# SenseTime-FVG/OpenDWM

Hardware: AMD Instinct MI355X
Metric: denoise-steps/sec (6-view x16f 448x256), SD-3.5 CTSD (higher is better)
Workload: dtype bf16; 1 GPU; CTSD SD-3.5 MMDiT (24 joint blocks, 13 dual, 6 cross-view + 12 temporal VT blocks, point-wise temporal + ImageAdapter), 6 views x 16 frames x 448x256 px (latents [1,16,6,16,32,56]), CFG g=4 -> model batch 2, 154 text tokens, FlowMatch-Euler; one replica per GPU; layers=24, finite=True, residual_stream=fp32 (GEMM operands and activations bf16), variant=text+layout (ImageAdapter recomputed every step, pointwise temporal)

## Files before the change

### include/dwm_hip.h

```cpp
#ifndef DWM_HIP_H
#define DWM_HIP_H

#include <stdint.h>

#ifdef __cplusplus
extern "C" {
#endif

#define DWM_OK 0
#define DWM_EINVAL (-1)
#define DWM_EALIGN (-2)
#define DWM_EUNSUPPORTED (-3)

#define DWM_ABI_VERSION 18
int dwm_abi_version(void);
const char* dwm_source_hash(void);

enum {
    DWM_EPI_PLAIN = 0,
    DWM_EPI_GEGLU = 1,
    DWM_EPI_RESID = 2,
    DWM_EPI_RMSHEAD = 3
};
enum { DWM_ACT_NONE = 0, DWM_ACT_GELU_TANH = 1, DWM_ACT_SILU = 2, DWM_ACT_RELU = 3 };

typedef struct dwm_rowmap2d {
    int64_t rw, rh;
    int64_t rpitch, ipitch;
    int64_t origin;
    int64_t xstep;
} dwm_rowmap2d;

typedef struct dwm_gemm_args {
    const void* A;  int64_t lda;
    const void* W;
    const void* bias;
    void* C;        int64_t ldc;
    int64_t M, N, K;
    int32_t epilogue;
    int32_t act;
    const void* gate; int64_t ld_gate; int64_t rows_per_gate;
    const void* res;  int64_t ld_res;  int64_t res_mod;
    const void* blend; int64_t ld_blend;
    const float* alpha; int64_t rows_per_alpha;
    const void* rms_w; int64_t rms_ncols; float rms_eps;
    int32_t reserved;
    dwm_rowmap2d a_map;
    dwm_rowmap2d c_map;
    int32_t ntaps; int32_t k_per_tap;
    int64_t tap_shift[27];
    void* workspace; int64_t workspace_bytes; int32_t split_k;
    void* C32; int64_t ldc32;
    int32_t tile;
} dwm_gemm_args;

int dwm_gemm_bf16(const dwm_gemm_args* args, void* stream);
int64_t dwm_gemm4w_launches(void);
int64_t dwm_gemm4w_launches_general(void);

typedef struct dwm_gemm_tn_args {
    const void* A; int64_t lda;
    const void* B; int64_t ldb; int64_t b_rows;
    void* out; int64_t ldo;
    int64_t M, N, C;
    int32_t ntaps; int32_t split_k;
    int64_t tap_shift[27];
    void* workspace; int64_t workspace_bytes;
} dwm_gemm_tn_args;
int dwm_gemm_tn(const dwm_gemm_tn_args* args, void* stream);

typedef struct dwm_attn_args {
    const void *q0, *k0, *v0; int64_t ld0;
    const void *q1, *k1, *v1; int64_t ld1;
    void* o0; int64_t ldo0;
    void* o1; int64_t ldo1;
    int64_t L0, L1;
    int64_t n_problems;
    int32_t heads; int32_t head_dim;
    float scale;
    int32_t mask_mode;
    int64_t pdiv[3], pmod[3], pstride[3];
    int64_t ldiv[2], lstride[3];
    const uint8_t* mask; int64_t mask_G; int64_t group_size; int64_t p_per_mask;
    int32_t variant;
    int32_t cross;
    float* lse;
} dwm_attn_args;

int dwm_attention_fwd(const dwm_attn_args* args, void* stream);
int64_t dwm_attn_stream_launches(void);

typedef struct dwm_attn_bwd_args {
    dwm_attn_args fwd;
    const void *do0, *do1;
    void *dq0, *dk0, *dv0; int64_t ld_d0;
    void *dq1, *dk1, *dv1; int64_t ld_d1;
    float* delta;
} dwm_attn_bwd_args;
int dwm_attention_bwd(const dwm_attn_bwd_args* args, void* stream);

int dwm_debug_tr_probe(const int32_t* offs, int16_t* out, void* stream);

typedef struct dwm_layernorm_args {
    const void* x; int64_t ldx;
    void* y;       int64_t ldy;
    void* y2;      int64_t ldy2;
    void* xsum;    int64_t ldxsum;
    int64_t rows; int32_t D; float eps;
    const void* weight; const void* bias;
    const void* scale;  const void* shift;  int64_t ld_mod;  int64_t rows_per_mod;
    const void* scale2; const void* shift2;
// ... 189 lines not shown
```

### opendwm_amd/_lib.py

```python
from __future__ import annotations

import ctypes as C
import os

HERE = os.path.dirname(os.path.abspath(__file__))
LIB_PATH = os.environ.get("DWM_HIP_LIB") or os.path.join(HERE, "libdwm_hip.so")
ABI_VERSION = 18

EPI_PLAIN, EPI_GEGLU, EPI_RESID, EPI_RMSHEAD = 0, 1, 2, 3
ACT_NONE, ACT_GELU_TANH, ACT_SILU, ACT_RELU = 0, 1, 2, 3

_i64, _i32, _f32, _vp = C.c_int64, C.c_int32, C.c_float, C.c_void_p


class RowMap2D(C.Structure):
    _fields_ = [("rw", _i64), ("rh", _i64), ("rpitch", _i64), ("ipitch", _i64), ("origin", _i64), ("xstep", _i64)]


class GemmTnArgs(C.Structure):
    _fields_ = [
        ("A", _vp), ("lda", _i64), ("B", _vp), ("ldb", _i64), ("b_rows", _i64), ("out", _vp), ("ldo", _i64),
        ("M", _i64), ("N", _i64), ("C", _i64), ("ntaps", _i32), ("split_k", _i32), ("tap_shift", _i64 * 27),
        ("workspace", _vp), ("workspace_bytes", _i64),
    ]
# ... 44 lines not shown
        ("weight", _vp), ("bias", _vp),
        ("scale", _vp), ("shift", _vp), ("ld_mod", _i64), ("rows_per_mod", _i64),
        ("scale2", _vp), ("shift2", _vp),
        ("addvec", _vp), ("ld_add", _i64), ("rows_per_add", _i64),
    ]


class GnImgMap(C.Structure):
    _fields_ = [("iv", _i64), ("pn", _i64), ("s_ihi", _i64), ("s_ilo", _i64), ("s_phi", _i64)]


class GnZMap(C.Structure):
    _fields_ = [("mod", _vp), ("ld_mod", _i64), ("frames", _i32), ("videos", _i32), ("h", _i32), ("w", _i32),
                ("shift", _i32), ("zt", _i32 * 32)]


class FrameMix(C.Structure):
    _fields_ = [("n_out", _i32), ("f0", _i32 * 64), ("f1", _i32 * 64), ("w0", _f32 * 64), ("w1", _f32 * 64)]


class BlockPermuteArgs(C.Structure):
    _fields_ = [("src", C.c_void_p), ("dst", C.c_void_p), ("block_bytes", C.c_int64), ("n", C.c_int64 * 4), ("sstride", C.c_int64 * 4)]


class RowCombineArgs(C.Structure):
    _fields_ = [
        ("a", _vp), ("lda", _i64), ("gate_a", _vp), ("ld_gate_a", _i64), ("rows_per_gate_a", _i64),
        ("coef_a", _vp), ("rows_per_coef_a", _i64), ("b", _vp), ("ldb", _i64),
        ("coef_b", _vp), ("rows_per_coef_b", _i64), ("out", _vp), ("ldo", _i64), ("rows", _i64), ("ncols", _i64),
    ]


class LayerNormBwdArgs(C.Structure):
    _fields_ = [
        ("x", _vp), ("ldx", _i64), ("addvec", _vp), ("ld_add", _i64), ("rows_per_add", _i64),
        ("dy", _vp), ("lddy", _i64), ("dy2", _vp), ("lddy2", _i64),
        ("dx", _vp), ("lddx", _i64), ("accumulate", _i32),
        ("rows", _i64), ("D", _i32), ("eps", _f32), ("weight", _vp),
        ("scale", _vp), ("scale2", _vp), ("ld_mod", _i64), ("rows_per_mod", _i64),
        ("dgamma", _vp), ("dbeta", _vp), ("dgamma2", _vp), ("dbeta2", _vp), ("ld_grad", _i64), ("grad_per_group", _i32),
    ]


class AdamW8Item(C.Structure):
    _fields_ = [("p", _vp), ("g", _vp), ("m_q", _vp), ("m_absmax", _vp), ("v_q", _vp), ("v_absmax", _vp), ("p_bf16", _vp), ("n", _i64)]


SIGNATURES = {
    "dwm_abi_version": (_i32, []),
    "dwm_source_hash": (C.c_char_p, []),
    "dwm_gemm_bf16": (_i32, [C.POINTER(GemmArgs), _vp]),
    "dwm_gemm4w_launches": (_i64, []),
    "dwm_gemm4w_launches_general": (_i64, []),
    "dwm_attn_stream_launches": (_i64, []),
    "dwm_gemm_tn": (_i32, [C.POINTER(GemmTnArgs), _vp]),
    "dwm_attention_fwd": (_i32, [C.POINTER(AttnArgs), _vp]),
    "dwm_attention_bwd": (_i32, [C.POINTER(AttnBwdArgs), _vp]),
    "dwm_debug_tr_probe": (_i32, [_vp, _vp, _vp]),
    "dwm_layernorm": (_i32, [C.POINTER(LayerNormArgs), _vp]),
    "dwm_layernorm_x32": (_i32, [C.POINTER(LayerNormArgs), _vp]),
    "dwm_rmsnorm_heads": (_i32, [_vp, _i64, _i64, _i64, _vp, _f32, _vp]),
    "dwm_silu": (_i32, [_vp, _vp, _i64, _vp]),
    "dwm_timestep_sinusoid": (_i32, [_vp, _i64, _i32, _vp, _vp]),
    "dwm_patchify": (_i32, [_vp, _i32, _i64, _i32, _i32, _i32, _i32, _vp, _i64, _vp]),
    "dwm_unpatchify": (_i32, [_vp, _i64, _i64, _i32, _i32, _i32, _i32, _vp, _vp]),
    "dwm_cfg_euler_step": (_i32, [_vp, _vp, _vp, _i64, _f32, _f32, _vp]),
    "dwm_cfg_euler_step_grouped": (_i32, [_vp, _vp, _vp, _i64, _f32, _vp, _i64, _vp]),
    "dwm_cast_f32_to_bf16": (_i32, [_vp, _vp, _i64, _vp]),
    "dwm_gemm_f32": (_i32, [C.POINTER(GemmArgs), _vp]),
    "dwm_layernorm_f32": (_i32, [C.POINTER(LayerNormArgs), _vp]),
    "dwm_groupnorm_silu_f32": (_i32, [_vp, _vp, _i64, _i64, _i32, _i32, _f32, _vp, _vp, _i32, _vp, C.POINTER(RowMap2D), C.POINTER(GnImgMap), _vp]),
    "dwm_upsample2_padded_f32": (_i32, [_vp, _vp, _i64, _i32, _i32, _i32, _vp]),
    "dwm_pad_tokens_f32": (_i32, [_vp, _vp, _i64, _i32, C.POINTER(RowMap2D), _vp]),
    "dwm_softmax_rows_f32": (_i32, [_vp, _vp, _i64, _i32, _i64, _f32, _vp]),
    "dwm_unshuffle_tokens_f32": (_i32, [_vp, _i64, _i32, _i32, _i32, _i32, _vp, _i64, _vp]),
    "dwm_avgpool2_tokens_f32": (_i32, [_vp, _i64, _i32, _i32, _i32, _vp, _vp]),
    "dwm_cfg_multistep_f32": (_i32, [_vp, _vp, _vp, _vp, _i64, _f32, _f32, _f32, _f32, _f32, _f32, _vp]),
    "dwm_attention_f32": (_i32, [C.POINTER(AttnArgs), _vp]),
    "dwm_silu_f32": (_i32, [_vp, _vp, _i64, _vp]),
    "dwm_timestep_sinusoid_f32": (_i32, [_vp, _i64, _i32, _vp, _vp]),
    "dwm_patchify_f32": (_i32, [_vp, _i64, _i32, _i32, _i32, _i32, _vp, _i64, _vp]),
    "dwm_unpatchify_f32": (_i32, [_vp, _i64, _i64, _i32, _i32, _i32, _i32, _vp, _vp]),
    "dwm_cfg_euler_step_f32": (_i32, [_vp, _vp, _vp, _i64, _f32, _f32, _vp, _i64, _vp]),
    "dwm_ray_features": (_i32, [_vp, _i64, _i32, _i32, _vp, _i64, _vp]),
    "dwm_ray_features_f32": (_i32, [_vp, _i64, _i32, _i32, _vp, _i64, _vp]),
    "dwm_frame_affine": (_i32, [_vp, _vp, _vp, _vp, _vp, _i64, _i64, _vp]),
    "dwm_cfg_ddim_step": (_i32, [_vp, _i32, _i32, _vp, _vp, _vp, _vp, _vp, _i64, _i64, _f32, _i32, _f32, _i32, _vp]),
    "dwm_cfg_multistep": (_i32, [_vp, _vp, _vp, _vp, _i64, _f32, _f32, _f32, _f32, _f32, _f32, _vp]),
    "dwm_unshuffle_tokens": (_i32, [_vp, _i32, _i64, _i32, _i32, _i32, _i32, _vp, _i64, _vp]),
    "dwm_avgpool2_tokens": (_i32, [_vp, _i64, _i32, _i32, _i32, _vp, _vp]),
    "dwm_add_inplace": (_i32, [_vp, _vp, _i64, _vp]),
    "dwm_add_f32_inplace": (_i32, [_vp, _vp, _i64, _vp]),
    "dwm_add_f32_f32_inplace": (_i32, [_vp, _vp, _i64, _vp]),
    "dwm_groupnorm_silu": (_i32, [_vp, _vp, _i64, _i64, _i32, _i32, _f32, _vp, _vp, _i32, _vp, C.POINTER(RowMap2D), _vp]),
    "dwm_groupnorm_silu_mapped": (_i32, [_vp, _vp, _i64, _i64, _i32, _i32, _f32, _vp, _vp, _i32, _vp, C.POINTER(RowMap2D), C.POINTER(GnImgMap), _vp]),
    "dwm_upsample2_padded": (_i32, [_vp, _vp, _i64, _i32, _i32, _i32, _vp]),
    "dwm_pad_tokens": (_i32, [_vp, _vp, _i64, _i32, C.POINTER(RowMap2D), _vp]),
    "dwm_groupnorm_stats_floats": (_i64, [_i64, _i64, _i32]),
    "dwm_groupnorm_spatial": (_i32, [_vp, _vp, _i64, _i64, _i32, _i32, _f32, _vp, _vp, _i32, _vp, C.POINTER(RowMap2D),
                                     C.POINTER(GnImgMap), C.POINTER(GnZMap), _vp]),
    "dwm_frame_mix_bf16": (_i32, [_vp, _vp, _i64, C.POINTER(FrameMix), _vp]),
    "dwm_frame_mix_f32": (_i32, [_vp, _vp, _i64, C.POINTER(FrameMix), _vp]),
    "dwm_groupnorm_spatial_f32": (_i32, [_vp, _vp, _i64, _i64, _i32, _i32, _f32, _vp, _vp, _i32, _vp, C.POINTER(RowMap2D),
                                         C.POINTER(GnImgMap), C.POINTER(GnZMap), _vp]),
    "dwm_softmax_rows": (_i32, [_vp, _vp, _i64, _i32, _i64, _f32, _vp]),
    "dwm_transpose_bf16": (_i32, [_vp, _i64, _i64, _i64, _vp, _i64, _i64, _vp]),
# ... 70 lines not shown
```

### opendwm_amd/build.py

```python
from __future__ import annotations

import os
import shutil
import subprocess
import sys
from concurrent.futures import ThreadPoolExecutor

HERE = os.path.dirname(os.path.abspath(__file__))
CSRC = os.path.join(HERE, "csrc")
INCLUDE = os.path.join(os.path.dirname(HERE), "include")
LIB = os.path.join(HERE, "libdwm_hip.so")
SOURCES = ["gemm_bf16.hip", "gemm_bf16_4w.hip", "gemm_tn.hip", "attention.hip", "attention_stream.hip", "attention_bwd.hip", "norm.hip",
           "elementwise.hip", "vae.hip", "train.hip", "fp32path.hip"]
AGPR_SOURCES: set = {"gemm_bf16_4w.hip", "attention_stream.hip"}
FILE_FLAGS: dict = {"attention_stream.hip": ["-fno-slp-vectorize"]}
VGPR_FORM = ["-mllvm", "-amdgpu-mfma-vgpr-form"]
ARCH = "gfx950"


def _hipcc() -> str:
    for c in (os.environ.get("HIPCC"), "/opt/rocm/bin/hipcc", shutil.which("hipcc")):
        if c and os.path.exists(c):
            return c
    raise RuntimeError("hipcc not found (need ROCm to build libdwm_hip.so)")


def _stale(target: str, deps) -> bool:
    if not os.path.exists(target):
        return True
    t = os.path.getmtime(target)
    return any(os.path.getmtime(d) > t for d in deps)


def source_hash() -> str:
    import hashlib
    h = hashlib.sha256()
    files = sorted(os.path.join(CSRC, f) for f in os.listdir(CSRC) if f.endswith((".hip", ".h"))) + [os.path.join(INCLUDE, "dwm_hip.h")]
    for f in files:
        h.update(os.path.basename(f).encode())
        h.update(open(f, "rb").read())
    return h.hexdigest()


def build(force: bool = False, verbose: bool = False) -> str:
    hipcc = _hipcc()
    headers = [os.path.join(CSRC, "common.h"), os.path.join(CSRC, "attention_common.h"), os.path.join(CSRC, "gemm_common.h"),
               os.path.join(INCLUDE, "dwm_hip.h")]
    shash = source_hash()
    stamp = os.path.join(CSRC, "build", ".source_hash")
    objdir = os.path.join(CSRC, "build")
    os.makedirs(objdir, exist_ok=True)
    base = [f"--offload-arch={ARCH}", "-O3", "-std=c++17", "-fPIC", "-fno-gpu-rdc", f"-I{INCLUDE}", f"-I{CSRC}"]
    user = os.environ.get("DWM_EXTRA_FLAGS", "").split()
    jobs = []
    extra = " ".join(os.environ.get("DWM_EXTRA_FLAGS", "").split())
    old_hash, old_extra = "", ""
    if os.path.exists(stamp):
        lines = open(stamp).read().split("\n")
        old_hash, old_extra = lines[0].strip(), (lines[1].strip() if len(lines) > 1 else "")
    force = force or old_extra != extra
    for src in SOURCES:
        s = os.path.join(CSRC, src)
        o = os.path.join(objdir, src.replace(".hip", ".o"))
        if force or _stale(o, [s] + headers) or (src == "elementwise.hip" and old_hash != shash):
            jobs.append((s, o))

    def compile_one(job):
# ... 44 lines not shown
```

### opendwm_amd/csrc/gemm_bf16.hip

```cpp
#include <cstdlib>
#include <type_traits>

#include "gemm_common.h"

namespace {

using namespace dwm_gemm;

#ifdef DWM_DEV_HOOKS
#define DWM_RESERVED(x_) (x_)
#define DWM_DEV_LDS_PAD 16384
#else
#define DWM_RESERVED(x_) 0
#define DWM_DEV_LDS_PAD 0
#endif

constexpr int BM = 256, BN = 256, BK = 64;
constexpr int TILE_BYTES = BM * BK * 2;
constexpr int A_STAGES = 3, W_STAGES = 2;
constexpr int W_BASE = A_STAGES * TILE_BYTES;
constexpr int LDS_BYTES = (A_STAGES + W_STAGES) * TILE_BYTES;

template <int TC> struct TileCfg;
template <> struct TileCfg<0> { static constexpr int bm = 256, bn = 256, bk = 64, nwn = 4, nwaves = 8, ast = A_STAGES, wst = W_STAGES; };
// ... 993 lines not shown
        case 3: return launch8w<DWM_EPI_RESID, true, true, 0, 3>(a, cp, pl, s);
        case 2: return launch8w<DWM_EPI_RESID, true, true, 0, 2>(a, cp, pl, s);
        default: return launch8w<DWM_EPI_RESID, true, true, 0, 6>(a, cp, pl, s);
    }
}
template <int TC>
int launch_resid_rs(const dwm_gemm_args& a, const ConvParams& cp, const GemmPlan& pl, hipStream_t s) {
    switch (pl.rs) {
        case 2: return launch8w<DWM_EPI_RESID, true, false, TC, 2>(a, cp, pl, s);
        case 3: return launch8w<DWM_EPI_RESID, true, false, TC, 3>(a, cp, pl, s);
        case 6: return launch8w<DWM_EPI_RESID, true, false, TC, 6>(a, cp, pl, s);
        default: return launch8w<DWM_EPI_RESID, true, false, TC, 18>(a, cp, pl, s);
    }
}
template <int EPI>
int launch_epi(const dwm_gemm_args& a, const ConvParams& cp, const GemmPlan& pl, hipStream_t s) {
    if (pl.fast) return pl.tc == 1 ? launch8w<EPI, true, false, 1, 0>(a, cp, pl, s) : launch8w<EPI, true, false, 0, 0>(a, cp, pl, s);
    return pl.tc == 1 ? launch8w<EPI, false, false, 1, 0>(a, cp, pl, s) : launch8w<EPI, false, false, 0, 0>(a, cp, pl, s);
}
int launch_tile(const dwm_gemm_args& a, const ConvParams& cp, const GemmPlan& pl, hipStream_t s) {
    if (pl.rs != 0) return pl.tc == 1 ? launch_resid_rs<1>(a, cp, pl, s) : launch_resid_rs<0>(a, cp, pl, s);
    switch (pl.epi) {
        case DWM_EPI_PLAIN: return launch_epi<DWM_EPI_PLAIN>(a, cp, pl, s);
        case DWM_EPI_GEGLU: return launch_epi<DWM_EPI_GEGLU>(a, cp, pl, s);
        case DWM_EPI_RESID: return launch_epi<DWM_EPI_RESID>(a, cp, pl, s);
        default: return launch_epi<DWM_EPI_RMSHEAD>(a, cp, pl, s);
    }
}

}

extern "C" int dwm_gemm_bf16(const dwm_gemm_args* a_in, void* stream) {
    if (a_in == nullptr) return DWM_EINVAL;
    const int tile_asked = a_in->tile;
    dwm_gemm_args a_copy;
    if (tile_asked == 3 || tile_asked == 4) { a_copy = *a_in; a_copy.tile = 0; }
    const dwm_gemm_args& a = tile_asked == 3 || tile_asked == 4 ? a_copy : *a_in;

    if (a.A == nullptr || a.W == nullptr || (a.C == nullptr && a.C32 == nullptr)) return DWM_EINVAL;
    int rc = check_sizes(a, kBf16);
    if (rc != DWM_OK) return rc;
    if (a.lda % 8 != 0 || (a.C != nullptr && a.ldc % 8 != 0)) return DWM_EALIGN;
    if (!dwm_aligned16(a.A) || !dwm_aligned16(a.W) || !dwm_aligned16(a.C)) return DWM_EALIGN;
    if (a.bias && (((uintptr_t)a.bias) & 7u)) return DWM_EALIGN;
    if (a.C != nullptr && a.ldc < gemm_nout(a)) return DWM_EINVAL;
    rc = check_epilogue(a, kBf16);
    if (rc != DWM_OK) return rc;
    if (a.C32 != nullptr && a.epilogue != DWM_EPI_RESID) return DWM_EUNSUPPORTED;

    GemmPlan plan;
    rc = plan_gemm(a, tile_asked, plan);
    if (rc != DWM_OK) return rc;
    hipStream_t s = (hipStream_t)stream;
    if (plan.family == GemmFamily::W4_FAST || plan.family == GemmFamily::W4_GENERAL) return dwm_gemm4w_launch(a, plan, s);
    ConvParams cp;
    fill_conv_params(a, plan, cp);
    switch (plan.family) {
        case GemmFamily::W8_SPLITK: return launch_splitk(a, cp, plan, s);
        case GemmFamily::W8_C32: return launch_c32(a, cp, plan, s);
        default: return launch_tile(a, cp, plan, s);
    }
}
```

### opendwm_amd/csrc/gemm_bf16_4w.hip

```cpp
#include <atomic>

#include "gemm_common.h"

namespace {

using namespace dwm_gemm;

typedef __attribute__((ext_vector_type(8))) __bf16 hbf16x8;
typedef __attribute__((ext_vector_type(4))) int i32x4;

constexpr int BM = 256, BN = 256, BK = 64;
constexpr int TILE = BM * BK * 2;
constexpr int AST = 3, WST = 2;
constexpr int W_BASE = AST * TILE;
constexpr int LDS_BYTES = (AST + WST) * TILE;
constexpr int NJ = TILE / (4 * 1024);

struct G4Params {
    int ntm, ntn, gm;
    FastDiv fd_rpg, fd_rpa;
    FastDiv fd_rmod;
    DevRowMap amap;
    int steps_per_tap;
    int64_t a_base_rows;
// ... 278 lines not shown
                f32x2 ss2 = {0.f, 0.f};
#pragma unroll
                for (int jj = 0; jj < 4; ++jj)
#pragma unroll
                    for (int r = 0; r < 4; r += 2) {
                        const f32x2 v = (f32x2){acc[i][4 * s + jj][r], acc[i][4 * s + jj][r + 1]} + (f32x2){bv[4 * s + jj][r], bv[4 * s + jj][r + 1]};
                        x[jj][r] = v[0]; x[jj][r + 1] = v[1];
                        ss2 += v * v;
                    }
                float ss = ss2[0] + ss2[1];
                ss += __shfl_xor(ss, 16, 64);
                ss += __shfl_xor(ss, 32, 64);
                const float rinv = do_norm[s] ? rsqrtf(ss * (1.f / 64.f) + p.rms_eps) : 1.f;
#pragma unroll
                for (int jj = 0; jj < 4; ++jj) {
                    float y[4];
#pragma unroll
                    for (int r = 0; r < 4; ++r) y[r] = x[jj][r] * rinv * rw[4 * s + jj][r];
                    const int b = 4 * s + jj;
                    *(uint2*)(scr + l15 * RB + (((2 * b + (lg >> 1)) ^ (l15 & (NCH - 1))) << 4) + (lg & 1) * 8) = pack4(y);
                }
            }
        } else if constexpr (kResid) {
#pragma unroll
            for (int j = 0; j < 8; ++j)
                *(float4*)(scr + l15 * RB + (((4 * j + lg) ^ l15) << 4)) = make_float4(acc[i][j][0], acc[i][j][1], acc[i][j][2], acc[i][j][3]);
        } else {
#define DWM4_ACT_PASS(FN_)                                                                                         \
            _Pragma("unroll") for (int j = 0; j < 8; ++j) {                                                        \
                float y[4];                                                                                        \
                _Pragma("unroll") for (int r = 0; r < 4; r += 2) {                                                 \
                    const f32x2 x = FN_((f32x2){acc[i][j][r], acc[i][j][r + 1]} + (f32x2){bv[j][r], bv[j][r + 1]}); \
                    y[r] = x[0]; y[r + 1] = x[1];                                                                  \
                }                                                                                                  \
                *(uint2*)(scr + l15 * RB + (((2 * j + (lg >> 1)) ^ (l15 & (NCH - 1))) << 4) + (lg & 1) * 8) = pack4(y); \
            }
            if (p.act == DWM_ACT_GELU_TANH) { DWM4_ACT_PASS(gelu_tanh2) }
            else if (p.act == DWM_ACT_SILU) { DWM4_ACT_PASS(silu2) }
            else if (p.act == DWM_ACT_RELU) { DWM4_ACT_PASS(relu2) }
            else { DWM4_ACT_PASS() }
#undef DWM4_ACT_PASS
        }
#pragma unroll
        for (int st = 0; st < NST; ++st) {
            const int r = st * RPS + rrow;
            const int64_t m = m0 + wm * 128 + i * 16 + r;
            if constexpr (!kResid) {
                const uint4 o = *(const uint4*)(scr + r * RB + ((rc8 ^ (r & (NCH - 1))) << 4));
                if (!GEN || (m < M && nok)) *(uint4*)((bf16_t*)p.C + ((uint64_t)(uint32_t)m * (uint32_t)p.ldc + (uint32_t)ocol)) = o;
            } else {
                const float4 x0 = *(const float4*)(scr + r * RB + (((2 * rc8) ^ r) << 4));
                const float4 x1 = *(const float4*)(scr + r * RB + (((2 * rc8 + 1) ^ r) << 4));
                float v[8] = {x0.x, x0.y, x0.z, x0.w, x1.x, x1.y, x1.z, x1.w};
                float t[8];
#pragma unroll
                for (int c = 0; c < 8; ++c) v[c] += b8[c];
                if constexpr (f_gate) {
                    unpack8(gA[st], t);
#pragma unroll
                    for (int c = 0; c < 8; ++c) v[c] *= t[c];
                }
                if constexpr (RF32) {
                    const float4 ta = *reinterpret_cast<const float4*>(&rA[st]), tb = *reinterpret_cast<const float4*>(&rB[st]);
                    t[0] = ta.x; t[1] = ta.y; t[2] = ta.z; t[3] = ta.w; t[4] = tb.x; t[5] = tb.y; t[6] = tb.z; t[7] = tb.w;
                } else {
                    unpack8(rA[st], t);
                }
#pragma unroll
                for (int c = 0; c < 8; ++c) v[c] += t[c];
                if constexpr (f_blend) {
                    if constexpr (RF32) {
                        const float4 ta = *reinterpret_cast<const float4*>(&blA[st]), tb = *reinterpret_cast<const float4*>(&blB[st]);
                        t[0] = ta.x; t[1] = ta.y; t[2] = ta.z; t[3] = ta.w; t[4] = tb.x; t[5] = tb.y; t[6] = tb.z; t[7] = tb.w;
                    } else {
                        unpack8(blA[st], t);
                    }
                    const float al = alA[st];
#pragma unroll
                    for (int c = 0; c < 8; ++c) v[c] = al * t[c] + (1.f - al) * v[c];
                }
                if (!GEN || (m < M && nok)) {
                    if constexpr (RF32) {
                        float* o32 = (float*)p.C32 + ((uint64_t)(uint32_t)m * (uint32_t)p.ldc32 + (uint32_t)ocol);
                        *(float4*)o32 = make_float4(v[0], v[1], v[2], v[3]);
                        *(float4*)(o32 + 4) = make_float4(v[4], v[5], v[6], v[7]);
                    } else {
                        *(uint4*)((bf16_t*)p.C + ((uint64_t)(uint32_t)m * (uint32_t)p.ldc + (uint32_t)ocol)) = pack8(v);
                    }
                }
            }
        }
        if (i + 1 < 8) issue_resid(i + 1);
    }
}

std::atomic<int64_t> g_launches{0};
std::atomic<int64_t> g_launches_gen{0};

template <int EPI, bool RF32, int RS, bool GEN = false>
int launch4w(const dwm_gemm_args& a, const G4Params& gp, hipStream_t s) {
    const hipError_t e = dwm_allow_dynamic_lds<gemm4w_kernel<EPI, RF32, RS, GEN>>(LDS_BYTES);
    if (e != hipSuccess) return (int)e;
    hipLaunchKernelGGL((gemm4w_kernel<EPI, RF32, RS, GEN>), dim3((unsigned)(gp.ntm * gp.ntn)), dim3(256), LDS_BYTES, s, a, gp);
    g_launches.fetch_add(1, std::memory_order_relaxed);
    if (GEN) g_launches_gen.fetch_add(1, std::memory_order_relaxed);
    return dwm_launch_status();
}
template <int EPI, bool RF32, int RS>
int launch4w_form(const dwm_gemm_args& a, const G4Params& gp, bool gen, hipStream_t s) {
    return gen ? launch4w<EPI, RF32, RS, true>(a, gp, s) : launch4w<EPI, RF32, RS, false>(a, gp, s);
}

void tap_span(const dwm_gemm_args& a, int64_t& smin, int64_t& smax) {
    smin = smax = 0;
    for (int t = 0; t < a.ntaps; ++t) {
        smin = a.tap_shift[t] < smin ? a.tap_shift[t] : smin;
        smax = a.tap_shift[t] > smax ? a.tap_shift[t] : smax;
    }
}

void fill_g4(const dwm_gemm_args& a, const GemmPlan& plan, G4Params& gp) {
    gp.ntm = plan.ntm; gp.ntn = plan.ntn;
    gp.gm = plan.gm;
    gp.fd_rpg = make_fastdiv((uint32_t)(a.rows_per_gate > 0 ? a.rows_per_gate : 1));
    gp.fd_rpa = make_fastdiv((uint32_t)(a.rows_per_alpha > 0 ? a.rows_per_alpha : 1));
    gp.fd_rmod = make_fastdiv((uint32_t)(a.res_mod < 0 ? -a.res_mod : 1));
    const dwm_rowmap2d identity = {};
    make_dev_rowmap(a.a_map.rw > 0 ? a.a_map : identity, gp.amap);
    gp.steps_per_tap = (int)(a.K / BK);
    gp.a_base_rows = 0;
    for (int t = 0; t < 27; ++t) gp.tap_off[t] = 0;
    if (plan.family != GemmFamily::W4_GENERAL) return;
    gp.steps_per_tap = (int)(gemm_k_per_tap(a) / BK);
    int64_t smin, smax;
    tap_span(a, smin, smax);
    gp.a_base_rows = smin;
    for (int t = 0; t < a.ntaps; ++t) gp.tap_off[t] = (uint32_t)((a.tap_shift[t] - smin) * a.lda * 2);
}

}

bool dwm_gemm4w_covers(const dwm_gemm_args& a, bool fast_only, GemmPlan& plan) {
    const int64_t lim = 1ll << 31;
    if (a.c_map.rw > 0 || a.split_k > 1 || a.K < 2 * BK) return false;
    const bool row_div = a.epilogue == DWM_EPI_RESID && a.res_mod < 0;
    const bool gen = a.a_map.rw > 0 || a.ntaps > 0 || a.M % BM != 0 || a.N % BN != 0 || row_div;
    if (gen && fast_only) return false;
    if (a.ldc >= lim || a.ldc32 >= lim || a.ld_res >= lim || a.ld_blend >= lim || a.ld_gate >= lim) return false;
    const int ntm = (int)((a.M + BM - 1) / BM), ntn = (int)((a.N + BN - 1) / BN);
    if (auto_splitk(a, (int64_t)ntm * ntn)) return false;
    int rs = 0;
    if (a.epilogue == DWM_EPI_RESID) {
        if (a.res_mod > 0 || a.act != DWM_ACT_NONE || a.res == nullptr) return false;
        rs = (a.gate ? 1 : 0) | 2 | (a.blend ? 4 : 0) | (row_div ? 16 : 0);
        if (a.C32 != nullptr && (a.C != nullptr || row_div)) return false;
        if (rs != 2 && rs != 3 && rs != 6 && !(rs == 18 && a.C32 == nullptr)) return false;
    } else if (a.C32 != nullptr) {
        return false;
    }
    if (!gen) {
        if (a.lda * 2 * BM >= lim || a.K * 2 * BN >= lim || a.lda * 2 >= (1ll << 28)) return false;
    } else {
        if (a.M >= (1ll << 30) || a.res_mod < -(1ll << 30) || a.rows_per_gate > (1ll << 30) || a.rows_per_alpha > (1ll << 30)) return false;
        const int ntaps = gemm_ntaps(a);
        const int64_t kpt = gemm_k_per_tap(a);
        if (ntaps > 27 || kpt <= 0 || kpt % BK != 0 || kpt * ntaps != a.K || a.lda < kpt) return false;
        DevRowMap amap;
        if (!make_dev_rowmap(a.a_map, amap)) return false;
        int64_t smin, smax;
        tap_span(a, smin, smax);
        int64_t last = a.M - 1;
        if (a.a_map.rw > 0) {
            const dwm_rowmap2d& r = a.a_map;
            const int64_t q = last / r.rw, x = last % r.rw, img = q / r.rh, y = q % r.rh;
            last = img * r.ipitch + y * r.rpitch + x * (r.xstep > 0 ? r.xstep : 1) + r.origin;
        }
        if (last < 0 || (last + smax - smin + 1) * a.lda * 2 + a.K * 2 >= lim || a.N * a.K * 2 >= lim) return false;
    }
    plan.family = gen ? GemmFamily::W4_GENERAL : GemmFamily::W4_FAST;
    plan.epi = a.epilogue; plan.rs = rs;
    plan.fast = !gen; plan.rf32 = a.C32 != nullptr;
    plan.tc = 0;
    plan.ntm = ntm; plan.ntn = ntn;
    plan.grid = (unsigned)(ntm * ntn); plan.block = 256; plan.lds = LDS_BYTES;
    plan.ksplit = 1;
    plan.gm = raster_group_height(a.K);
    return true;
}

int dwm_gemm4w_launch(const dwm_gemm_args& a, const GemmPlan& plan, hipStream_t s) {
    G4Params gp;
    fill_g4(a, plan, gp);
    const bool gen = plan.family == GemmFamily::W4_GENERAL;
    switch (plan.epi) {
        case DWM_EPI_PLAIN: return launch4w_form<DWM_EPI_PLAIN, false, 0>(a, gp, gen, s);
        case DWM_EPI_GEGLU: return launch4w_form<DWM_EPI_GEGLU, false, 0>(a, gp, gen, s);
        case DWM_EPI_RMSHEAD: return launch4w_form<DWM_EPI_RMSHEAD, false, 0>(a, gp, gen, s);
        default: break;
    }
    if (plan.rf32) {
        if (plan.rs == 2) return launch4w_form<DWM_EPI_RESID, true, 2>(a, gp, gen, s);
        if (plan.rs == 3) return launch4w_form<DWM_EPI_RESID, true, 3>(a, gp, gen, s);
        return launch4w_form<DWM_EPI_RESID, true, 6>(a, gp, gen, s);
    }
    if (plan.rs == 2) return launch4w_form<DWM_EPI_RESID, false, 2>(a, gp, gen, s);
    if (plan.rs == 3) return launch4w_form<DWM_EPI_RESID, false, 3>(a, gp, gen, s);
    if (plan.rs == 6) return launch4w_form<DWM_EPI_RESID, false, 6>(a, gp, gen, s);
    return launch4w<DWM_EPI_RESID, false, 18, true>(a, gp, s);
}

extern "C" int64_t dwm_gemm4w_launches(void) { return g_launches.load(std::memory_order_relaxed); }
extern "C" int64_t dwm_gemm4w_launches_general(void) { return g_launches_gen.load(std::memory_order_relaxed); }
```

### opendwm_amd/csrc/gemm_common.h

```cpp
#pragma once
#include "common.h"
#include "dwm_hip.h"

namespace dwm_gemm {

struct DevRowMap {
    FastDiv rw, rh;
    int64_t rpitch, ipitch, origin;
    int enabled, xstep;
};
static inline bool make_dev_rowmap(const dwm_rowmap2d& r, DevRowMap& d) {
    d.enabled = r.rw > 0;
    d.xstep = r.xstep > 0 ? (int)r.xstep : 1;
    if (!d.enabled) { d.rw = make_fastdiv(1); d.rh = make_fastdiv(1); d.rpitch = d.ipitch = d.origin = 0; return true; }
    if (r.rh <= 0 || r.rw >= (1ll << 30) || r.rh >= (1ll << 30)) return false;
    d.rw = make_fastdiv((uint32_t)r.rw); d.rh = make_fastdiv((uint32_t)r.rh);
    d.rpitch = r.rpitch; d.ipitch = r.ipitch; d.origin = r.origin;
    return true;
}
DWM_DEVINL int64_t map_row(const DevRowMap& rm, int64_t m) {
    if (!rm.enabled) return m;
    const uint32_t q = fdiv((uint32_t)m, rm.rw), x = (uint32_t)m - q * rm.rw.d;
    const uint32_t i = fdiv(q, rm.rh), y = q - i * rm.rh.d;
    return (int64_t)i * rm.ipitch + (int64_t)y * rm.rpitch + (int64_t)x * rm.xstep + rm.origin;
}

enum class GemmFamily {
    W4_FAST,
    W4_GENERAL,
    W8_SPLITK,
    W8_256,
    W8_128,
    W8_C32
};
struct GemmPlan {
    GemmFamily family;
    int epi, rs;
    bool fast, rf32;
    int tc;
    int ntm, ntn;
    unsigned grid, block;
    int lds;
    int ksplit;
    int gm;
};

static inline int raster_group_height(int64_t K) { return K >= 4096 ? 4 : 8; }

static inline int64_t gemm_nout(const dwm_gemm_args& a) { return a.epilogue == DWM_EPI_GEGLU ? a.N / 2 : a.N; }
static inline int gemm_ntaps(const dwm_gemm_args& a) { return a.ntaps > 0 ? a.ntaps : 1; }
static inline int64_t gemm_k_per_tap(const dwm_gemm_args& a) { return a.ntaps > 0 ? a.k_per_tap : a.K; }

static inline bool splitk_pays(int64_t tiles, int64_t nk) { return tiles <= 128 && nk >= 16; }
static inline bool auto_splitk(const dwm_gemm_args& a, int64_t tiles) {
    return (a.epilogue == DWM_EPI_PLAIN || a.epilogue == DWM_EPI_RESID) && a.workspace != nullptr && a.split_k == 0 &&
           a.C32 == nullptr && splitk_pays(tiles, a.K / 64);
}
static inline int clamp_ksplit(int ksplit, int64_t nk, int max_ranges, int64_t range_bytes, int64_t avail) {
    if (ksplit > nk / 8) ksplit = (int)(nk / 8);
    if (ksplit > max_ranges) ksplit = max_ranges;
    if ((int64_t)ksplit * range_bytes > avail) ksplit = (int)(avail / range_bytes);
    return ksplit;
}

}

bool dwm_gemm4w_covers(const dwm_gemm_args& a, bool fast_only, dwm_gemm::GemmPlan& plan);
int dwm_gemm4w_launch(const dwm_gemm_args& a, const dwm_gemm::GemmPlan& plan, hipStream_t s);
```

Baseline: 2.529 denoise-steps/s.

## Add persistent ping-pong wave-group GEMM for large fp32-residual epilogue GEMMs

Adds a persistent 512-thread GEMM kernel that splits a 256x256 tile into two 128-column halves handled by two wave groups. One group runs MFMA compute while the other runs the fp32 residual/gate/blend epilogue, swapping roles each slot, fed by a 6-deep buffer_load-to-LDS ring. The planner sends fp32-residual GEMMs with at least 512 tiles to this kernel, aiming to hide epilogue memory traffic behind compute. In exchange it adds heavy hand-written barrier choreography and a single-block-per-CU launch bound.

```diff
diff --git a/include/dwm_hip.h b/include/dwm_hip.h
--- a/include/dwm_hip.h
+++ b/include/dwm_hip.h
@@ -57,6 +57,7 @@
 int dwm_gemm_bf16(const dwm_gemm_args* args, void* stream);
 int64_t dwm_gemm4w_launches(void);
 int64_t dwm_gemm4w_launches_general(void);
+int64_t dwm_gemm4w_pair_launches(void);
 
 typedef struct dwm_gemm_tn_args {
     const void* A; int64_t lda;
diff --git a/opendwm_amd/_lib.py b/opendwm_amd/_lib.py
--- a/opendwm_amd/_lib.py
+++ b/opendwm_amd/_lib.py
@@ -120,6 +120,7 @@
     "dwm_gemm_bf16": (_i32, [C.POINTER(GemmArgs), _vp]),
     "dwm_gemm4w_launches": (_i64, []),
     "dwm_gemm4w_launches_general": (_i64, []),
+    "dwm_gemm4w_pair_launches": (_i64, []),
     "dwm_attn_stream_launches": (_i64, []),
     "dwm_gemm_tn": (_i32, [C.POINTER(GemmTnArgs), _vp]),
     "dwm_attention_fwd": (_i32, [C.POINTER(AttnArgs), _vp]),
diff --git a/opendwm_amd/build.py b/opendwm_amd/build.py
--- a/opendwm_amd/build.py
+++ b/opendwm_amd/build.py
@@ -10,9 +10,9 @@
 CSRC = os.path.join(HERE, "csrc")
 INCLUDE = os.path.join(os.path.dirname(HERE), "include")
 LIB = os.path.join(HERE, "libdwm_hip.so")
-SOURCES = ["gemm_bf16.hip", "gemm_bf16_4w.hip", "gemm_tn.hip", "attention.hip", "attention_stream.hip", "attention_bwd.hip", "norm.hip",
+SOURCES = ["gemm_bf16.hip", "gemm_bf16_4w.hip", "gemm_bf16_4w_pair.hip", "gemm_tn.hip", "attention.hip", "attention_stream.hip", "attention_bwd.hip", "norm.hip",
            "elementwise.hip", "vae.hip", "train.hip", "fp32path.hip"]
-AGPR_SOURCES: set = {"gemm_bf16_4w.hip", "attention_stream.hip"}
+AGPR_SOURCES: set = {"gemm_bf16_4w.hip", "gemm_bf16_4w_pair.hip", "attention_stream.hip"}
 FILE_FLAGS: dict = {"attention_stream.hip": ["-fno-slp-vectorize"]}
 VGPR_FORM = ["-mllvm", "-amdgpu-mfma-vgpr-form"]
 ARCH = "gfx950"
diff --git a/opendwm_amd/csrc/gemm_bf16.hip b/opendwm_amd/csrc/gemm_bf16.hip
--- a/opendwm_amd/csrc/gemm_bf16.hip
+++ b/opendwm_amd/csrc/gemm_bf16.hip
@@ -1069,7 +1069,7 @@
     rc = plan_gemm(a, tile_asked, plan);
     if (rc != DWM_OK) return rc;
     hipStream_t s = (hipStream_t)stream;
-    if (plan.family == GemmFamily::W4_FAST || plan.family == GemmFamily::W4_GENERAL) return dwm_gemm4w_launch(a, plan, s);
+    if (plan.family == GemmFamily::W4_FAST || plan.family == GemmFamily::W4_GENERAL || plan.family == GemmFamily::W4_PAIR) return dwm_gemm4w_launch(a, plan, s);
     ConvParams cp;
     fill_conv_params(a, plan, cp);
     switch (plan.family) {
diff --git a/opendwm_amd/csrc/gemm_bf16_4w.hip b/opendwm_amd/csrc/gemm_bf16_4w.hip
--- a/opendwm_amd/csrc/gemm_bf16_4w.hip
+++ b/opendwm_amd/csrc/gemm_bf16_4w.hip
@@ -354,33 +354,7 @@
                 const float4 x0 = *(const float4*)(scr + r * RB + (((2 * rc8) ^ r) << 4));
                 const float4 x1 = *(const float4*)(scr + r * RB + (((2 * rc8 + 1) ^ r) << 4));
                 float v[8] = {x0.x, x0.y, x0.z, x0.w, x1.x, x1.y, x1.z, x1.w};
-                float t[8];
-#pragma unroll
-                for (int c = 0; c < 8; ++c) v[c] += b8[c];
-                if constexpr (f_gate) {
-                    unpack8(gA[st], t);
-#pragma unroll
-                    for (int c = 0; c < 8; ++c) v[c] *= t[c];
-                }
-                if constexpr (RF32) {
-                    const float4 ta = *reinterpret_cast<const float4*>(&rA[st]), tb = *reinterpret_cast<const float4*>(&rB[st]);
-                    t[0] = ta.x; t[1] = ta.y; t[2] = ta.z; t[3] = ta.w; t[4] = tb.x; t[5] = tb.y; t[6] = tb.z; t[7] = tb.w;
-                } else {
-                    unpack8(rA[st], t);
-                }
-#pragma unroll
-                for (int c = 0; c < 8; ++c) v[c] += t[c];
-                if constexpr (f_blend) {
-                    if constexpr (RF32) {
-                        const float4 ta = *reinterpret_cast<const float4*>(&blA[st]), tb = *reinterpret_cast<const float4*>(&blB[st]);
-                        t[0] = ta.x; t[1] = ta.y; t[2] = ta.z; t[3] = ta.w; t[4] = tb.x; t[5] = tb.y; t[6] = tb.z; t[7] = tb.w;
-                    } else {
-                        unpack8(blA[st], t);
-                    }
-                    const float al = alA[st];
-#pragma unroll
-                    for (int c = 0; c < 8; ++c) v[c] = al * t[c] + (1.f - al) * v[c];
-                }
+                resid_row8<f_gate, f_blend, RF32>(v, b8, gA[st], rA[st], rB[st], blA[st], blB[st], alA[st]);
                 if (!GEN || (m < M && nok)) {
                     if constexpr (RF32) {
                         float* o32 = (float*)p.C32 + ((uint64_t)(uint32_t)m * (uint32_t)p.ldc32 + (uint32_t)ocol);
@@ -487,10 +461,19 @@
     plan.grid = (unsigned)(ntm * ntn); plan.block = 256; plan.lds = LDS_BYTES;
     plan.ksplit = 1;
     plan.gm = raster_group_height(a.K);
+    if (!gen && !fast_only && plan.rf32 && pair_pays((int64_t)ntm * ntn, a.K) && a.M * a.lda * 2 < lim && a.N * a.K * 2 < lim) {
+        plan.family = GemmFamily::W4_PAIR;
+        const int ncu = dwm_cu_count();
+        plan.grid = (unsigned)(ntm * ntn < ncu ? ntm * ntn : ncu); plan.block = 512;
+    }
     return true;
 }
 
 int dwm_gemm4w_launch(const dwm_gemm_args& a, const GemmPlan& plan, hipStream_t s) {
+    if (plan.family == GemmFamily::W4_PAIR) {
+        g_launches.fetch_add(1, std::memory_order_relaxed);
+        return dwm_gemm4w_pair_launch(a, plan, s);
+    }
     G4Params gp;
     fill_g4(a, plan, gp);
     const bool gen = plan.family == GemmFamily::W4_GENERAL;
diff --git a/opendwm_amd/csrc/gemm_bf16_4w_pair.hip b/opendwm_amd/csrc/gemm_bf16_4w_pair.hip
--- /dev/null
+++ b/opendwm_amd/csrc/gemm_bf16_4w_pair.hip
@@ -0,0 +1,290 @@
+#include <atomic>
+
+#include "gemm_common.h"
+
+namespace {
+
+using namespace dwm_gemm;
+
+typedef __attribute__((ext_vector_type(8))) __bf16 hbf16x8;
+typedef __attribute__((ext_vector_type(4))) int i32x4;
+
+constexpr int BM = 256, BN = 256, BNH = 128, BK = 32;
+constexpr int A_BYTES = BM * BK * 2;
+constexpr int W_BYTES = BNH * BK * 2;
+constexpr int STAGE = A_BYTES + W_BYTES;
+constexpr int RING = 6, AHEAD = RING - 1;
+constexpr int SCR_BASE = RING * STAGE;
+constexpr int LDS_BYTES = SCR_BASE + 4 * 4096;
+constexpr int NJA = 4, NJW = 2, NJ = NJA + NJW;
+
+struct PairParams {
+    int ntm, ntn, gm;
+    FastDiv fd_rpg, fd_rpa;
+};
+
+template <int RS>
+__global__ void __launch_bounds__(512, 1)
+gemm4w_pair_kernel(const dwm_gemm_args p, const PairParams gp) {
+    static_assert(RS == 2 || RS == 3 || RS == 6, "residual / gate + residual / residual + blend");
+    constexpr bool f_gate = (RS & 1) != 0, f_blend = (RS & 4) != 0;
+    constexpr int NL = (f_gate ? 2 : 0) + 4 + (f_blend ? 6 : 0);
+    constexpr int PF = f_blend ? 2 : 3;
+    extern __shared__ __attribute__((aligned(16))) char smem[];
+    const int tid = threadIdx.x, lane = tid & 63;
+    const int wave8 = __builtin_amdgcn_readfirstlane(tid >> 6);
+    const int grp = wave8 >> 2, wave = wave8 & 3;
+    const int wm = wave >> 1, wn = wave & 1;
+    const int l15 = lane & 15, lg = lane >> 4;
+    const int64_t K = p.K;
+    const int nk = (int)(K / BK);
+    const int ntm = gp.ntm, ntn = gp.ntn, gm = gp.gm;
+    const int ntiles = ntm * ntn;
+    const int T = (ntiles - (int)blockIdx.x + (int)gridDim.x - 1) / (int)gridDim.x;
+    const int nslots = 2 * T;
+
+    auto tile_of = [&](int i, int& m0, int& n0) {
+        const int id = xcd_remap((int)blockIdx.x + i * (int)gridDim.x, ntiles);
+        const int per_group = gm * ntn;
+        const int g = id / per_group, in_grp = id - g * per_group;
+        const int first_m = g * gm;
+        const int gsize = ntm - first_m < gm ? ntm - first_m : gm;
+        m0 = __builtin_amdgcn_readfirstlane((first_m + in_grp % gsize) * BM);
+        n0 = __builtin_amdgcn_readfirstlane((in_grp / gsize) * BN);
+    };
+
+    auto make_rsrc = [](const void* ptr) {
+        const uint64_t a = (uint64_t)ptr;
+        i32x4 r;
+        r[0] = __builtin_amdgcn_readfirstlane((int)(uint32_t)a);
+        r[1] = __builtin_amdgcn_readfirstlane((int)(uint32_t)((a >> 32) & 0xffffu));
+        r[2] = -1;
+        r[3] = 0x00020000;
+        return r;
+    };
+    const i32x4 rs_a = make_rsrc(p.A), rs_w = make_rsrc(p.W);
+    const uint32_t chd = (uint32_t)((lane & 3) ^ ((4 - (lane >> 4)) & 3)) * 16u;
+    const uint32_t voff_a = (uint32_t)(wave * (NJA * 16) + (lane >> 2)) * (uint32_t)(p.lda * 2) + chd;
+    const uint32_t voff_w = (uint32_t)(wave * (NJW * 16) + (lane >> 2)) * (uint32_t)(K * 2) + chd;
+    const uint32_t step_a = 16u * (uint32_t)(p.lda * 2), step_w = 16u * (uint32_t)(K * 2);
+    const uint32_t lds0 = (uint32_t)(uintptr_t)(const __attribute__((address_space(3))) char*)smem;
+    auto bufld = [&](const i32x4& rs, uint32_t vo, uint32_t so) {
+        asm volatile("buffer_load_dwordx4 %0, %1, %2 offen lds\n\ts_add_u32 m0, m0, 0x400" ::"v"(vo), "s"(rs), "s"(so) : "memory", "m0");
+    };
+    auto set_m0 = [&](uint32_t lds_off) { asm volatile("s_mov_b32 m0, %0\n\ts_nop 0" ::"s"(lds0 + lds_off) : "memory", "m0"); };
+    int c_slot = 0, c_kt = 0, c_ring = 0;
+    uint32_t c_a = 0, c_w = 0;
+    auto cursor_coords = [&]() {
+        const int sl = c_slot < nslots ? c_slot : nslots - 1;
+        int m0, n0;
+        tile_of(sl >> 1, m0, n0);
+        c_a = (uint32_t)m0 * (uint32_t)(p.lda * 2);
+        c_w = (uint32_t)(n0 + (sl & 1) * BNH) * (uint32_t)(K * 2);
+    };
+    auto cursor_step = [&]() {
+        c_ring = c_ring == RING - 1 ? 0 : c_ring + 1;
+        if (++c_kt == nk) { c_kt = 0; ++c_slot; cursor_coords(); }
+    };
+    auto request = [&](int q) {
+        if (q == 0) set_m0((uint32_t)(c_ring * STAGE + wave * (NJA * 1024)));
+        if (q == NJA) set_m0((uint32_t)(c_ring * STAGE + A_BYTES + wave * (NJW * 1024)));
+        if (q < NJA) bufld(rs_a, voff_a, c_a + (uint32_t)c_kt * (BK * 2) + (uint32_t)q * step_a);
+        else bufld(rs_w, voff_w, c_w + (uint32_t)c_kt * (BK * 2) + (uint32_t)(q - NJA) * step_w);
+    };
+
+    const int coff = (lg ^ ((4 - (l15 >> 2)) & 3)) << 4;
+    const int a_row = (wm * 128 + l15) * (BK * 2) + coff, w_row = A_BYTES + (wn * 64 + l15) * (BK * 2) + coff;
+    hbf16x8 af[2][8], wf[2][4];
+    auto read_frags = [&](auto set_tag, int ring_slot) {
+        constexpr int S = decltype(set_tag)::value;
+        const char* st = smem + ring_slot * STAGE;
+#pragma unroll
+        for (int f = 0; f < 4; ++f) wf[S][f] = *(const hbf16x8*)(st + w_row + f * 1024);
+#pragma unroll
+        for (int f = 0; f < 8; ++f) af[S][f] = *(const hbf16x8*)(st + a_row + f * 1024);
+    };
+
+    f32x4 acc[8][4];
+    auto zero_acc = [&]() {
+#pragma unroll
+        for (int i = 0; i < 8; ++i)
+#pragma unroll
+            for (int j = 0; j < 4; ++j) {
+                acc[i][j] = (f32x4){0.f, 0.f, 0.f, 0.f};
+                asm volatile("" : "+a"(acc[i][j]));
+            }
+    };
+    auto barrier = [&]() {
+        __builtin_amdgcn_s_barrier();
+        asm volatile("" ::: "memory");
+    };
+
+    int ring = 0;
+
+    auto k_step = [&](auto b_tag, auto last_tag) {
+        constexpr int B = decltype(b_tag)::value;
+        constexpr bool LAST = decltype(last_tag)::value;
+        const int nxt = ring == RING - 1 ? 0 : ring + 1;
+        const char* sn = smem + nxt * STAGE;
+#pragma unroll
+        for (int i = 0; i < 8; ++i) {
+#pragma unroll
+            for (int j = 0; j < 4; ++j) {
+                acc[i][j] = __builtin_amdgcn_mfma_f32_16x16x32_bf16(wf[B][j], af[B][i], acc[i][j], 0, 0, 0);
+                const int idx = i * 4 + j;
+                if (!LAST) {
+                    if (idx < 4) wf[B ^ 1][idx] = *(const hbf16x8*)(sn + w_row + idx * 1024);
+                    else if (idx < 12) af[B ^ 1][idx - 4] = *(const hbf16x8*)(sn + a_row + (idx - 4) * 1024);
+                }
+                if (idx >= 12 && idx < 12 + 3 * NJ && (idx - 12) % 3 == 0) request((idx - 12) / 3);
+                __builtin_amdgcn_sched_barrier(0);
+            }
+        }
+        cursor_step();
+        ring = nxt;
+        asm volatile("s_waitcnt vmcnt(%0) lgkmcnt(0)" ::"n"(3 * NJ) : "memory");
+        barrier();
+    };
+    auto compute_slot = [&]() {
+        for (int kt = 0; kt + 2 < nk; kt += 2) {
+            k_step(std::integral_constant<int, 0>{}, std::false_type{});
+            k_step(std::integral_constant<int, 1>{}, std::false_type{});
+        }
+        k_step(std::integral_constant<int, 0>{}, std::false_type{});
+        k_step(std::integral_constant<int, 1>{}, std::true_type{});
+    };
+
+    char* const scr = smem + SCR_BASE + wave * 4096;
+    const int rrow = lane >> 3, rc8 = lane & 7;
+    uint4 gA[PF][2], rA[PF][2], rB[PF][2], blA[PF][2], blB[PF][2];
+    float alA[PF][2];
+    uint4 braw;
+    int em0 = 0, en0 = 0;
+    auto issue_resid = [&](auto set_tag, int i) {
+        constexpr int S = decltype(set_tag)::value;
+        const uint32_t ocol = (uint32_t)(en0 + wn * 64 + rc8 * 8);
+#pragma unroll
+        for (int st = 0; st < 2; ++st) {
+            const uint32_t m = (uint32_t)(em0 + wm * 128 + i * 16 + st * 8 + rrow);
+            if constexpr (f_gate) gA[S][st] = *(const uint4*)((const bf16_t*)p.gate + ((uint64_t)fdiv(m, gp.fd_rpg) * (uint32_t)p.ld_gate + ocol));
+            const float* rp = (const float*)p.res + ((uint64_t)m * (uint32_t)p.ld_res + ocol);
+            rA[S][st] = *(const uint4*)rp;
+            rB[S][st] = *(const uint4*)(rp + 4);
+            if constexpr (f_blend) {
+                const float* bp = (const float*)p.blend + ((uint64_t)m * (uint32_t)p.ld_blend + ocol);
+                blA[S][st] = *(const uint4*)bp;
+                blB[S][st] = *(const uint4*)(bp + 4);
+                alA[S][st] = p.alpha[fdiv(m, gp.fd_rpa)];
+            }
+        }
+    };
+    auto epi_pass = [&](auto i_tag) {
+        constexpr int i = decltype(i_tag)::value, S = i % PF;
+#pragma unroll
+        for (int j = 0; j < 4; ++j)
+            *(float4*)(scr + l15 * 256 + (((4 * j + lg) ^ l15) << 4)) = make_float4(acc[i][j][0], acc[i][j][1], acc[i][j][2], acc[i][j][3]);
+        const uint32_t ocol = (uint32_t)(en0 + wn * 64 + rc8 * 8);
+        float b8[8];
+        unpack8(braw, b8);
+#pragma unroll
+        for (int st = 0; st < 2; ++st) {
+            const int r = st * 8 + rrow;
+            const uint32_t m = (uint32_t)(em0 + wm * 128 + i * 16 + r);
+            const float4 x0 = *(const float4*)(scr + r * 256 + (((2 * rc8) ^ r) << 4));
+            const float4 x1 = *(const float4*)(scr + r * 256 + (((2 * rc8 + 1) ^ r) << 4));
+            float v[8] = {x0.x, x0.y, x0.z, x0.w, x1.x, x1.y, x1.z, x1.w};
+            resid_row8<f_gate, f_blend, true>(v, b8, gA[S][st], rA[S][st], rB[S][st], blA[S][st], blB[S][st], alA[S][st]);
+            float* o32 = (float*)p.C32 + ((uint64_t)m * (uint32_t)p.ldc32 + ocol);
+            *(float4*)o32 = make_float4(v[0], v[1], v[2], v[3]);
+            *(float4*)(o32 + 4) = make_float4(v[4], v[5], v[6], v[7]);
+        }
+        if constexpr (i + PF < 8) issue_resid(std::integral_constant<int, S>{}, i + PF);
+    };
+    auto memory_slot = [&](auto epi_tag) {
+        constexpr bool do_epi = decltype(epi_tag)::value;
+        if constexpr (do_epi) {
+            braw = make_uint4(0u, 0u, 0u, 0u);
+            if (p.bias != nullptr) braw = *(const uint4*)((const bf16_t*)p.bias + (en0 + wn * 64 + rc8 * 8));
+            issue_resid(std::integral_constant<int, 0>{}, 0);
+            issue_resid(std::integral_constant<int, 1>{}, 1);
+            if constexpr (PF > 2) issue_resid(std::integral_constant<int, 2>{}, 2);
+        }
+        if constexpr (do_epi) asm volatile("s_waitcnt vmcnt(%0)" ::"n"(2 * NJ + PF * NL) : "memory");
+        else asm volatile("s_waitcnt vmcnt(%0)" ::"n"(2 * NJ) : "memory");
+        barrier();
+        if constexpr (do_epi) asm volatile("s_waitcnt vmcnt(%0)" ::"n"(NJ + PF * NL) : "memory");
+        else asm volatile("s_waitcnt vmcnt(%0)" ::"n"(NJ) : "memory");
+        barrier();
+        if constexpr (do_epi) asm volatile("s_waitcnt vmcnt(%0)" ::"n"(PF * NL) : "memory");
+        else asm volatile("s_waitcnt vmcnt(0)" ::: "memory");
+        barrier();
+        const int n1 = nk - 4;
+        auto pass = [&](auto i_tag) {
+            constexpr int i = decltype(i_tag)::value;
+            const int c = (((i + 1) * n1) >> 3) - ((i * n1) >> 3);
+            for (int b = 0; b < c; ++b) barrier();
+            if constexpr (do_epi) epi_pass(i_tag);
+        };
+        pass(std::integral_constant<int, 0>{}); pass(std::integral_constant<int, 1>{});
+        pass(std::integral_constant<int, 2>{}); pass(std::integral_constant<int, 3>{});
+        pass(std::integral_constant<int, 4>{}); pass(std::integral_constant<int, 5>{});
+        pass(std::integral_constant<int, 6>{}); pass(std::integral_constant<int, 7>{});
+        zero_acc();
+        ++c_slot;
+        cursor_coords();
+        c_ring = (c_ring + nk) % RING;
+        ring = (ring + nk) % RING;
+        read_frags(std::integral_constant<int, 0>{}, ring);
+        asm volatile("s_waitcnt lgkmcnt(0)" ::: "memory");
+        barrier();
+    };
+
+    cursor_coords();
+#pragma unroll 1
+    for (int st = 0; st < AHEAD; ++st) {
+        if (grp == 0) {
+#pragma unroll
+            for (int q = 0; q < NJ; ++q) request(q);
+        }
+        cursor_step();
+    }
+    zero_acc();
+    asm volatile("s_waitcnt vmcnt(%0)" ::"n"(3 * NJ) : "memory");
+    barrier();
+    if (grp == 0) read_frags(std::integral_constant<int, 0>{}, 0);
+
+    if (grp == 1) memory_slot(std::false_type{});
+#pragma unroll 1
+    for (int t = 0; t < T; ++t) {
+        compute_slot();
+        tile_of(t, em0, en0);
+        en0 += grp * BNH;
+        memory_slot(std::true_type{});
+    }
+    if (grp == 0) memory_slot(std::false_type{});
+}
+
+std::atomic<int64_t> g_pair_launches{0};
+
+template <int RS>
+int launch_pair(const dwm_gemm_args& a, const PairParams& gp, unsigned grid, hipStream_t s) {
+    const hipError_t e = dwm_allow_dynamic_lds<gemm4w_pair_kernel<RS>>(LDS_BYTES);
+    if (e != hipSuccess) return (int)e;
+    hipLaunchKernelGGL((gemm4w_pair_kernel<RS>), dim3(grid), dim3(512), LDS_BYTES, s, a, gp);
+    g_pair_launches.fetch_add(1, std::memory_order_relaxed);
+    return dwm_launch_status();
+}
+
+}
+
+int dwm_gemm4w_pair_launch(const dwm_gemm_args& a, const GemmPlan& plan, hipStream_t s) {
+    PairParams gp;
+    gp.ntm = plan.ntm; gp.ntn = plan.ntn; gp.gm = plan.gm;
+    gp.fd_rpg = make_fastdiv((uint32_t)(a.rows_per_gate > 0 ? a.rows_per_gate : 1));
+    gp.fd_rpa = make_fastdiv((uint32_t)(a.rows_per_alpha > 0 ? a.rows_per_alpha : 1));
+    if (plan.rs == 2) return launch_pair<2>(a, gp, plan.grid, s);
+    if (plan.rs == 3) return launch_pair<3>(a, gp, plan.grid, s);
+    return launch_pair<6>(a, gp, plan.grid, s);
+}
+
+extern "C" int64_t dwm_gemm4w_pair_launches(void) { return g_pair_launches.load(std::memory_order_relaxed); }
diff --git a/opendwm_amd/csrc/gemm_common.h b/opendwm_amd/csrc/gemm_common.h
--- a/opendwm_amd/csrc/gemm_common.h
+++ b/opendwm_amd/csrc/gemm_common.h
@@ -28,6 +28,7 @@
 enum class GemmFamily {
     W4_FAST,
     W4_GENERAL,
+    W4_PAIR,
     W8_SPLITK,
     W8_256,
     W8_128,
@@ -52,6 +53,7 @@
 static inline int64_t gemm_k_per_tap(const dwm_gemm_args& a) { return a.ntaps > 0 ? a.k_per_tap : a.K; }
 
 static inline bool splitk_pays(int64_t tiles, int64_t nk) { return tiles <= 128 && nk >= 16; }
+static inline bool pair_pays(int64_t tiles, int64_t K) { (void)K; return tiles >= 512; }
 static inline bool auto_splitk(const dwm_gemm_args& a, int64_t tiles) {
     return (a.epilogue == DWM_EPI_PLAIN || a.epilogue == DWM_EPI_RESID) && a.workspace != nullptr && a.split_k == 0 &&
            a.C32 == nullptr && splitk_pays(tiles, a.K / 64);
@@ -63,7 +65,39 @@
     return ksplit;
 }
 
+template <bool GATE, bool BLEND, bool RF32>
+DWM_DEVINL void resid_row8(float (&v)[8], const float (&b8)[8], const uint4& g, const uint4& ra, const uint4& rb, const uint4& bla,
+                           const uint4& blb, float al) {
+    float t[8];
+#pragma unroll
+    for (int c = 0; c < 8; ++c) v[c] += b8[c];
+    if constexpr (GATE) {
+        unpack8(g, t);
+#pragma unroll
+        for (int c = 0; c < 8; ++c) v[c] *= t[c];
+    }
+    if constexpr (RF32) {
+        const float4 ta = *reinterpret_cast<const float4*>(&ra), tb = *reinterpret_cast<const float4*>(&rb);
+        t[0] = ta.x; t[1] = ta.y; t[2] = ta.z; t[3] = ta.w; t[4] = tb.x; t[5] = tb.y; t[6] = tb.z; t[7] = tb.w;
+    } else {
+        unpack8(ra, t);
+    }
+#pragma unroll
+    for (int c = 0; c < 8; ++c) v[c] += t[c];
+    if constexpr (BLEND) {
+        if constexpr (RF32) {
+            const float4 ta = *reinterpret_cast<const float4*>(&bla), tb = *reinterpret_cast<const float4*>(&blb);
+            t[0] = ta.x; t[1] = ta.y; t[2] = ta.z; t[3] = ta.w; t[4] = tb.x; t[5] = tb.y; t[6] = tb.z; t[7] = tb.w;
+        } else {
+            unpack8(bla, t);
+        }
+#pragma unroll
+        for (int c = 0; c < 8; ++c) v[c] = al * t[c] + (1.f - al) * v[c];
+    }
+}
+
 }
 
 bool dwm_gemm4w_covers(const dwm_gemm_args& a, bool fast_only, dwm_gemm::GemmPlan& plan);
 int dwm_gemm4w_launch(const dwm_gemm_args& a, const dwm_gemm::GemmPlan& plan, hipStream_t s);
+int dwm_gemm4w_pair_launch(const dwm_gemm_args& a, const dwm_gemm::GemmPlan& plan, hipStream_t s);
```

After: 2.257 denoise-steps/s. -10.7%, worse.
